# neevparikh/rpt

Hardware: AMD Instinct MI355X
Metric: Msamples/sec (higher is better)
Workload: dtype f32; 1 GPU; C3 lampshade-in-fog path trace 1024x1024x256spp; scene=examples/volumetric_pathtrace_lampshade.rs, parallelism=tile-shard x1, streams=2

## Files before the change

__graft_entry__.py:

```python
import os
import subprocess
import sys

ROOT = os.path.dirname(os.path.abspath(__file__))
if ROOT not in sys.path:
    sys.path.insert(0, ROOT)

HIPCC = os.environ.get("HIPCC", "/opt/rocm/bin/hipcc")
CSRC = os.path.join(ROOT, "rpt_amd", "csrc")
LIB = os.path.join(ROOT, "rpt_amd", "librpt_hip.so")


def _stale(target, sources):
    if not os.path.exists(target):
        return True
    t = os.path.getmtime(target)
    return any(os.path.getmtime(s) > t for s in sources)


def _digest(paths):
    import hashlib
    h = hashlib.sha256()
    for p in paths:
        with open(p, "rb") as f:
            h.update(f.read())
    return h.hexdigest()


SRCS = [os.path.join(CSRC, f) for f in ("kernels.hip", "kernels_f64.hip", "photon.hip", "rpt_capi.cpp", "rpt_comm.cpp")]
DEPS = SRCS + [os.path.join(CSRC, f) for f in ("device_core.h", "gpu_layout.h", "kernels.h", "host_internal.h", "f64_layout.h", "sort_scan.h")] + [
    os.path.join(ROOT, "include", "rpt_hip.h")]


FLAGS = ["--offload-arch=gfx950", "-O3", "-std=c++17", "-fno-slp-vectorize", "-fPIC", "-shared", "-Wl,-rpath,/opt/rocm/lib"]


FILE_FLAGS = {"kernels_f64.hip": ["-mllvm", "-disable-machine-licm"]}


def library_source_digest():
    import hashlib
    return hashlib.sha256((_digest(DEPS) + " ".join(FLAGS) + repr(sorted(FILE_FLAGS.items()))).encode()).hexdigest()


def _object_digest(src):
# ... 58 lines not shown
```

include/rpt_hip.h:

```cpp
#ifndef RPT_HIP_H
#define RPT_HIP_H

#include <stdint.h>

#ifdef __cplusplus
extern "C" {
#endif

#define RPT_OK 0
#define RPT_ERR_INVALID (-1)
#define RPT_ERR_STATE (-2)
#define RPT_ERR_DEVICE (-3)
#define RPT_ERR_UNSUPPORTED (-4)

typedef struct rpt_scene rpt_scene;

enum { RPT_SHAPE_SPHERE = 0, RPT_SHAPE_CUBE = 1, RPT_SHAPE_PLANE = 2, RPT_SHAPE_MESH = 3,
       RPT_SHAPE_GROUP = 4,
       RPT_SHAPE_MONOMIAL = 5  };

typedef struct rpt_shape_desc {
    int32_t kind;
    int32_t has_transform;
    double transform[16];
// ... 121 lines not shown
int rpt_debug_rng_u32(uint64_t seed, uint32_t pixel, uint32_t sample, uint32_t n, uint32_t* out);
int rpt_debug_material_sample_f(const rpt_material*, uint64_t n, const float* normals, const float* wos,
                                uint64_t seed, float* wi, float* pdf, int32_t* some);
int rpt_debug_material_bsdf(const rpt_material*, uint64_t n, const float* normals, const float* wos,
                            const float* wis, float* out_rgb);
int rpt_debug_radix_sort(uint64_t n, const uint64_t* keys, uint64_t* keys_out, uint32_t* order_out);
int rpt_debug_exclusive_scan2(uint64_t n, const uint32_t* a, const uint32_t* b, uint32_t* out_a, uint32_t* out_b, uint64_t totals[2]);
int rpt_debug_photon_positions64(rpt_scene*, double* out, uint64_t capacity);
int rpt_debug_photon_selections(rpt_scene*, uint32_t* out, uint64_t capacity_words, uint64_t dims[3]);
int rpt_debug_camera_rays(const rpt_camera*, const rpt_render_params*, uint64_t seed, uint32_t sample,
                          float* origins, float* dirs);
int rpt_debug_camera_sample(const rpt_camera*, const rpt_render_params*, uint64_t seed, uint32_t sample,
                            float* origins, float* dirs, uint32_t* next_word);
int rpt_debug_camera_sample_f64(const rpt_camera*, const rpt_render_params*, uint64_t seed, uint32_t sample,
                                double* origins, double* dirs, uint32_t* next_word);
int rpt_debug_light_sample(rpt_scene*, uint32_t light, uint64_t n, const float* positions, uint64_t seed, float* v, float* nrm,
                           float* pdf, float* intensity, float* wi, float* dist, uint32_t* next_word);
int rpt_debug_light_sample_f64(rpt_scene*, uint32_t light, uint64_t n, const double* positions, uint64_t seed, double* v, double* nrm,
                               double* pdf, double* intensity, double* wi, double* dist, uint32_t* next_word);
int rpt_debug_env_color(rpt_scene*, uint64_t n, const float* dirs, float* rgb);
int rpt_debug_env_color_f64(rpt_scene*, uint64_t n, const double* dirs, double* rgb);
int rpt_debug_medium_distance(rpt_scene*, uint64_t n, uint64_t seed, float* dmed, float* t_limit);
int rpt_debug_shadow_test(rpt_scene*, uint32_t light, uint64_t n, const float* origins, const float* dirs, const float* dist,
                          int32_t* out_flag, float* out_t);
int rpt_shadow_scan_info(rpt_scene*, uint32_t light, uint32_t out[4]);
int rpt_debug_distance_pair(float sigma_t, uint32_t k0, uint32_t n, float* out_new, float* out_guarded);

int rpt_debug_bounce(const rpt_material* m, uint32_t max_bounces, uint32_t depth, int32_t in_medium, int32_t medium_event,
                     float albedo_med, const float* medium_color, uint64_t n, const float* normals, const float* rds, uint64_t seed,
                     int32_t* flag, float* wi, float* k, uint32_t* next_word);
// ... 9 lines not shown
```

rpt_amd/_lib.py:

```python
import ctypes as C
import os
import sys

_HERE = os.path.dirname(os.path.abspath(__file__))
LIB_PATH = os.environ.get("RPT_LIB", os.path.join(_HERE, "librpt_hip.so"))


class RptError(RuntimeError):
    """Raised for every non-zero return code of the C ABI (message from rpt_last_error)."""


class ShapeDesc(C.Structure):
    pass


ShapeDesc._fields_ = [
    ("kind", C.c_int32),
    ("has_transform", C.c_int32),
    ("transform", C.c_double * 16),
    ("plane_normal", C.c_double * 3),
    ("plane_value", C.c_double),
    ("tris", C.POINTER(C.c_double)),
    ("n_tris", C.c_uint64),
    ("children", C.POINTER(ShapeDesc)),
# ... 105 lines not shown
     [C.POINTER(MaterialDesc), C.c_uint64, _P, _P, C.c_uint64, _P, _P, _P]),
    ("rpt_debug_material_bsdf", C.c_int, [C.POINTER(MaterialDesc), C.c_uint64, _P, _P, _P, _P]),
    ("rpt_debug_radix_sort", C.c_int, [C.c_uint64, _P, _P, _P]),
    ("rpt_debug_exclusive_scan2", C.c_int, [C.c_uint64, _P, _P, _P, _P, C.POINTER(C.c_uint64)]),
    ("rpt_debug_photon_positions64", C.c_int, [_P, _P, C.c_uint64]),
    ("rpt_debug_photon_selections", C.c_int, [_P, _P, C.c_uint64, C.POINTER(C.c_uint64)]),
    ("rpt_debug_camera_rays", C.c_int,
     [C.POINTER(CameraDesc), C.POINTER(RenderParams), C.c_uint64, C.c_uint32, _P, _P]),
    ("rpt_debug_light_sample", C.c_int, [_P, C.c_uint32, C.c_uint64, _P, C.c_uint64, _P, _P, _P, _P, _P, _P, _P]),
    ("rpt_debug_light_sample_f64", C.c_int, [_P, C.c_uint32, C.c_uint64, _P, C.c_uint64, _P, _P, _P, _P, _P, _P, _P]),
    ("rpt_debug_env_color", C.c_int, [_P, C.c_uint64, _P, _P]),
    ("rpt_debug_env_color_f64", C.c_int, [_P, C.c_uint64, _P, _P]),
    ("rpt_debug_medium_distance", C.c_int, [_P, C.c_uint64, C.c_uint64, _P, _P]),
    ("rpt_debug_camera_sample", C.c_int,
     [C.POINTER(CameraDesc), C.POINTER(RenderParams), C.c_uint64, C.c_uint32, _P, _P, _P]),
    ("rpt_debug_camera_sample_f64", C.c_int,
     [C.POINTER(CameraDesc), C.POINTER(RenderParams), C.c_uint64, C.c_uint32, _P, _P, _P]),
    ("rpt_debug_bounce", C.c_int, [C.POINTER(MaterialDesc), C.c_uint32, C.c_uint32, C.c_int32, C.c_int32, C.c_float, _P,
                                   C.c_uint64, _P, _P, C.c_uint64, _P, _P, _P, _P]),
    ("rpt_debug_shadow_test", C.c_int, [_P, C.c_uint32, C.c_uint64, _P, _P, _P, _P, _P]),
    ("rpt_debug_distance_pair", C.c_int, [C.c_float, C.c_uint32, C.c_uint32, _P, _P]),
    ("rpt_shadow_scan_info", C.c_int, [_P, C.c_uint32, C.POINTER(C.c_uint32)]),
    ("rpt_debug_material_f64", C.c_int, [C.POINTER(MaterialDesc), C.c_uint64, _P, _P, C.c_uint64, _P, _P, _P, _P, _P]),
    ("rpt_debug_material_bsdf_f64", C.c_int, [C.POINTER(MaterialDesc), C.c_uint64, _P, _P, _P, _P]),
]

_lib = None


def vp(a):
# ... 28 lines not shown
```

rpt_amd/api.py:

```python
import ctypes as C
import math
import weakref

import numpy as np

from . import _lib
from ._lib import RptError, vp as _vp

def shard_pixels(width, height, rank, count):
    lib = _lib.load()
    n = _lib.check(lib.rpt_shard_tiles(width, height, rank, count, None, 0))
    tiles = np.zeros(max(n, 1), dtype=np.uint32)
    _lib.check(lib.rpt_shard_tiles(width, height, rank, count, tiles.ctypes.data_as(C.c_void_p), n))
    tiles_x = (width + 31) // 32
    ys, xs = np.mgrid[0:32, 0:32]
    out = []
    for t in tiles[:n]:
        x = (int(t) % tiles_x) * 32 + xs
        y = (int(t) // tiles_x) * 32 + ys
        m = (x < width) & (y < height)
        out.append((y[m] * width + x[m]).astype(np.uint32))
    return np.sort(np.concatenate(out)) if out else np.zeros(0, dtype=np.uint32)


# ... 900 lines not shown
        o = np.ascontiguousarray(origins, dtype=np.float32).reshape(-1, 3)
        d = np.ascontiguousarray(dirs, dtype=np.float32).reshape(-1, 3)
        ds = np.ascontiguousarray(dist, dtype=np.float32).reshape(-1)
        n = o.shape[0]
        if d.shape[0] != n or ds.shape[0] != n:
            raise ValueError("origins, dirs and dist differ in length")
        flag, t = np.empty(n, np.int32), np.empty(n, np.float32)
        _lib.check(lib.rpt_debug_shadow_test(h, light_index, n, _vp(o), _vp(d), _vp(ds), _vp(flag), _vp(t)))
        return flag, t

    def shadow_scan_info(self, light_index):
        out = (C.c_uint32 * 4)()
        _lib.check(_lib.load().rpt_shadow_scan_info(self.scene._commit(self.device_), light_index, out))
        return {"twin_lo": int(out[0]), "twin_hi": int(out[1]), "shadow_form": int(out[2]), "twin_object": int(np.int32(np.uint32(out[3])))}


def debug_distance_pair(sigma_t, k0, n):
    new, guarded = np.empty(n, np.float32), np.empty(n, np.float32)
    _lib.check(_lib.load().rpt_debug_distance_pair(float(sigma_t), int(k0), int(n), _vp(new), _vp(guarded)))
    return new, guarded


def debug_bounce(material, normals, rds, max_bounces=3, depth=0, seed=0, in_medium=False, medium_event=False, albedo_med=0.0,
                 medium_color=(0.0, 0.0, 0.0)):
    nrm = np.ascontiguousarray(normals, dtype=np.float32).reshape(-1, 3)
    rd = np.ascontiguousarray(rds, dtype=np.float32).reshape(-1, 3)
    n = nrm.shape[0]
    if rd.shape[0] != n:
        raise ValueError("normals and rds differ in length")
    mcol = np.ascontiguousarray(medium_color, dtype=np.float32).reshape(3)
# ... 29 lines not shown
    md = material_desc(material, _lib.MaterialDesc)
    _lib.check(_lib.load().rpt_debug_material_bsdf_f64(C.byref(md), n, *[_vp(a) for a in arrs], _vp(f)))
    return f


def debug_camera_sample(camera, width, height, sample=0, seed=0, f64=False):
    ft = np.float64 if f64 else np.float32
    n = width * height
    out = {"o": np.empty((n, 3), ft), "d": np.empty((n, 3), ft), "next_word": np.empty(n, np.uint32)}
    prm = _lib.RenderParams(width, height, 0.0, 0, 0, 1)
    lib = _lib.load()
    fn = lib.rpt_debug_camera_sample_f64 if f64 else lib.rpt_debug_camera_sample
    _lib.check(fn(C.byref(camera_desc(camera, _lib.CameraDesc)), C.byref(prm), seed, sample,
                  *[_vp(out[k]) for k in ("o", "d", "next_word")]))
    return out
```

rpt_amd/csrc/kernels.h:

```cpp
#pragma once
#include <hip/hip_runtime_api.h>
#include <stddef.h>
#include <stdint.h>
#include "gpu_layout.h"

namespace rptg {

struct RenderArgs {
    SceneView sc;
    CameraG cam;
    uint32_t width, height;
    float inv_dim;
    uint32_t max_bounces;
    uint32_t iterations;
    uint32_t sample_offset;
    uint32_t chunk_spp;
    uint32_t n_chunks;
    uint64_t seed_mixed;
    const uint32_t* tiles;
    uint32_t n_tiles, tiles_x;
    uint32_t n_owned;
    uint32_t n_items;
    float* slab;
    float* slab2;
    unsigned long long* queue;
    unsigned long long* counters;
    uint32_t lds_stack;
    uint32_t defer_lanes;
    uint32_t defer_stop;
    uint32_t walk_leaf_quarters;
    uint32_t detach;
    uint32_t pull_batch;
    uint32_t detach_trigger;
    uint32_t stream_backlog;
    uint32_t stream_contexts;
    uint32_t n_twin_lights;
    uint32_t* stream_scratch;
};

static_assert(offsetof(RenderArgs, sc) == 0, "RenderArgs must begin with the SceneView");

struct KernelInfo {
// ... 15 lines not shown
hipError_t launch_frame_unpack(const double* d_packed, double* d_frame, const uint32_t* d_tiles, uint32_t n_tiles, uint32_t tiles_x,
                               uint32_t width, uint32_t height, hipStream_t st);
__attribute__((weak)) hipError_t launch_intersect_segments(const SceneView& sc, uint64_t n, const float* d_o, const float* d_d, const float* d_tmax,
                                                           float* d_t, uint32_t* d_code, hipStream_t stream);
hipError_t launch_intersect(const SceneView& sc, uint64_t n, const float* d_o, const float* d_d, float* d_t,
                            int32_t* d_obj, float* d_n, bool bvh, hipStream_t stream);
hipError_t launch_debug_rng(uint64_t seed_mixed, uint32_t pixel, uint32_t sample, uint32_t n, uint32_t* d_out,
                            hipStream_t stream);
hipError_t launch_debug_sample_f(const Material& m, uint64_t n, const float* d_n, const float* d_wo,
                                 uint64_t seed_mixed, float* d_wi, float* d_pdf, int32_t* d_some, hipStream_t s);
hipError_t launch_debug_bsdf(const Material& m, uint64_t n, const float* d_n, const float* d_wo, const float* d_wi,
                             float* d_out, hipStream_t s);
__attribute__((weak)) hipError_t launch_debug_camera_sample(const CameraG& cam, uint32_t w, uint32_t h, float inv_dim, uint64_t seed_mixed,
                                                            uint32_t sample, float* d_o, float* d_d, uint32_t* d_next_word ,
                                                            hipStream_t s);
struct LightSampleArgs {
    uint32_t light;
    uint32_t pad_;
    uint64_t n;
    uint64_t seed_mixed;
    const float* pos;
    float *v, *nrm, *pdf;
    float *intensity, *wi, *dist;
    uint32_t* next_word;
};
__attribute__((weak)) hipError_t launch_debug_light_sample(const SceneView& sc, const LightSampleArgs& q, hipStream_t s);
__attribute__((weak)) hipError_t launch_debug_env_color(const SceneView& sc, uint64_t n, const float* d_dirs, float* d_rgb, hipStream_t s);
__attribute__((weak)) hipError_t launch_debug_medium_distance(const SceneView& sc, uint64_t n, uint64_t seed_mixed, float* d_dmed,
                                                              float* d_limit, hipStream_t s);
struct ShadowTestArgs {
// ... 38 lines not shown
```

rpt_amd/csrc/kernels.hip:

```cpp
#include "device_core.h"
#include "kernels.h"

namespace rptg {

RPT_DEV uint32_t mbcnt64(uint64_t m) {
    return __builtin_amdgcn_mbcnt_hi(uint32_t(m >> 32), __builtin_amdgcn_mbcnt_lo(uint32_t(m), 0u));
}
template <bool MONO = false>
RPT_DEV uint32_t code_object(const SceneView& sc, uint32_t code, uint32_t inst) {
    uint32_t kind = code >> 28, idx = code & 0x0FFFFFFFu;
    float w;
    if (MONO && kind == K_MONO) w = sc.mono_sh[idx].r0.w;
    else if (kind == K_INSTTRI) w = sc.inst[inst].n0.w;
    else if (kind == K_SPHERE) w = sc.sph_sh[idx].r0.w;
    else if (kind == K_CUBE) w = sc.cub_sh[idx].r0.w;
    else if (kind == K_PLANE) w = sc.pln_sh[idx].unit_n_obj.w;
    else if (kind == K_TRI) w = sc.tri_sh[idx].n1.w;
    else if (kind == K_AABB) w = sc.aabb[idx].lo.w;
    else if (kind == K_RECT) w = sc.rect_sh[idx].n_obj.w;
    else w = sc.btri_sh[idx].n1.w;
    return __float_as_uint(w);
}
RPT_DEV float ray_tmin(V o) { return 2e-5f * (1.f + max3(fabsf(o.x), fabsf(o.y), fabsf(o.z))); }

// ... 181 lines not shown
        if (bounce) {
            float pdf;
            SECT(13);
            const V wo = -normalize(rd);
            bounce = sample_f(mat, n, wo, rng, wi, pdf);
            if (bounce) {
                V f = bsdf(mat, n, wo, wi);
                float wgt = fabsf(dot(wi, n)) * rcp(MEDIUM ? pdf * 0.8f : pdf);
                k = wgt * f;
            }
        }
    }
    return bounce && !is_zero(k);
}

template <bool MEDIUM, int BVH, bool COUNT, bool GROUPS = false, int DETACH = 0, bool MONO = false>
__global__ __launch_bounds__(256, BVH == 0 ? ((GROUPS || COUNT || MONO) ? RPT_MIN_WAVES_SCAN_GROUPS : RPT_MIN_WAVES_SCAN) : BVH == 3 ? RPT_MIN_WAVES_SCENE_MESH : BVH == 1 ? (DETACH == 2 ? RPT_MIN_WAVES_STREAM : RPT_MIN_WAVES_MESH) : RPT_MIN_WAVES)
void render_kernel(const RenderArgs a) {
#ifdef RPT_SECT_CLOCKS
    __shared__ unsigned long long sect_lds_[4][56];
    if ((threadIdx.x & 63u) < 56u) sect_lds_[threadIdx.x >> 6][threadIdx.x & 63u] = 0ull;
    uint64_t sect_clk_ = __builtin_amdgcn_s_memtime();
    uint32_t sect_prev_ = 27u;
#endif
    static_assert(DETACH == 0 || (MEDIUM && BVH == 1 && !GROUPS), "detached tree walks: per-mesh-tree kernels in a medium only");
    static_assert(DETACH == 0 || !MONO, "no detached tree walks in scenes with monomial surfaces");
    extern __shared__ uint32_t dyn_lds[];
    const SceneView& sc = a.sc;
    uint32_t* stk = BVH ? (dyn_lds + threadIdx.x) : nullptr;
    const uint32_t stride = 256;

    const float sigma_t = sc.sigma_a + sc.sigma_s;
    const float inv_sigma_t = MEDIUM ? 1.f / sigma_t : 0.f;
    const float albedo_med = MEDIUM ? sc.sigma_s / sigma_t : 0.f;

    Rng rng;
    rng.s0 = rng.s1 = rng.s2 = rng.s3 = 0;
    V ro = mk(0, 0, 0), rd = mk(0, 0, 1);
    V P = mk(0, 0, 0), Q = mk(1, 1, 1), Rc = mk(kInf, kInf, kInf);
    constexpr uint32_t kStackRows = BVH == 1 ? (DETACH ? kDetachStackRows : 21u) : 32u;
    constexpr uint32_t kStateBase = BVH ? kStackRows * 256u : 0u;
    uint32_t* const ls = dyn_lds + kStateBase + threadIdx.x;
    enum { S_SLAB = 0, S_END = 1, S_PIX = 2, S_XN = 3, S_YN = 4, S_S = 5, S_ACC = 6, S_P = 9, S_Q = 12, S_RC = 15, S_ROWS = 18 };
    static_assert(S_RC + 3 == S_ROWS, "the staged tables begin right behind the state rows");
    constexpr uint32_t kTabBase = kStateBase + (BVH == 0 ? uint32_t(S_ROWS) : 5u) * 256u;
    LdsTables tab;
    {
        const F4* const t4 = reinterpret_cast<const F4*>(dyn_lds + kTabBase);
        F4* const w4 = reinterpret_cast<F4*>(dyn_lds + kTabBase);
        const uint32_t nm = sc.n_obj <= kLdsMats ? sc.n_obj : 0u, nl = sc.n_ltris <= kLdsLtris ? sc.n_ltris : 0u;
        for (uint32_t i = threadIdx.x; i < 2u * nm; i += 256u) w4[i] = reinterpret_cast<const F4*>(sc.mats)[i];
        for (uint32_t i = threadIdx.x; i < 6u * nl; i += 256u) w4[2u * kLdsMats + i] = reinterpret_cast<const F4*>(sc.ltris)[i];
        __syncthreads();
        tab.mats = t4; tab.n_mats = nm;
        tab.ltris = t4 + 2u * kLdsMats; tab.n_ltris = nl;
    }
    auto in_lds = [](int k) { return BVH == 0 || k <= S_YN; };
    V acc_r = mk(0, 0, 0);
    uint32_t slab_idx_r = 0, s_r = 0, s_end_r = 0, pix_r = 0;
// ... 87 lines not shown
        const uint32_t n_want = uint32_t(__popcll(__ballot(want)));
        if (n_want != 0u && (n_want >= a.pull_batch || __ballot(alive && !want) == 0ull)) {
            const auto& ka = *kernarg_args<RenderArgs>();
            SECTK(0);
            if (want && have_item) {
                if constexpr (DETACH) {
                    const volatile unsigned long long* av = acc64;
                    reinterpret_cast<float4*>(ka.slab)[ldu(S_SLAB, slab_idx_r)] =
                        make_float4(from_fixed(av[threadIdx.x]), from_fixed(av[256u + threadIdx.x]), from_fixed(av[512u + threadIdx.x]), 0.f);
                } else {
                    reinterpret_cast<float4*>(ka.slab)[ldu(S_SLAB, slab_idx_r)] =
                        make_float4(ldf(S_ACC + 0, acc_r.x), ldf(S_ACC + 1, acc_r.y), ldf(S_ACC + 2, acc_r.z), 0.f);
                }
                have_item = false;
            }
            for (;;) {
                const uint64_t m = __ballot(want);
                if (m == 0) break;
                if (pool_next == pool_end) {
                    unsigned long long base = ~0ull;
                    if (first_batch) {
                        base = (unsigned long long)(blockIdx.x * 4u + (threadIdx.x >> 6)) * 64ull;
                        first_batch = false;
                    } else if (!drained && (threadIdx.x & 63u) == 0) {
                        base = atomicAdd(ka.queue, 64ull);
                    }
                    const uint32_t lo = __builtin_amdgcn_readfirstlane(uint32_t(base));
                    const uint32_t hi = __builtin_amdgcn_readfirstlane(uint32_t(base >> 32));
                    if (hi != 0 || lo >= ka.n_items) {
                        drained = true;
                        if (want) alive = false;
                        break;
                    }
                    pool_next = lo;
                    pool_end = min(lo + 64u, ka.n_items);
                    pool_chunk = lo / ka.n_owned;
                    const uint32_t p0 = lo - pool_chunk * ka.n_owned;
// ... 14 lines not shown
                    if (x < ka.width && y < ka.height) {
                        want = false;
                        have_item = true;
                        item_done = false;
                        stu(S_SLAB, slab_idx_r, item);
                        if constexpr (DETACH) {
                            volatile unsigned long long* av = acc64;
                            av[threadIdx.x] = 0ull; av[256u + threadIdx.x] = 0ull; av[512u + threadIdx.x] = 0ull;
                        } else {
                            stf(S_ACC + 0, acc_r.x, 0.f);
                            stf(S_ACC + 1, acc_r.y, 0.f);
                            stf(S_ACC + 2, acc_r.z, 0.f);
                        }
                        const uint32_t s0 = chunk * ka.chunk_spp;
                        stu(S_S, s_r, s0);
                        stu(S_END, s_end_r, min(s0 + ka.chunk_spp, ka.iterations));
                        stu(S_PIX, pix_r, y * ka.width + x);
                        stf(S_XN, xn_r, pixel_xn(x, ka.width, ka.inv_dim));
                        stf(S_YN, yn_r, pixel_yn(y, ka.height, ka.inv_dim));
                    }
                }
            }
        }
        if (need_path && alive && !item_done && !(DETACH == 2 && uint32_t(__popc(parked_mask)) >= a.stream_contexts)) {
            if (alive) {
                const auto& ka = *kernarg_args<RenderArgs>();
                SECTK(1);
                const uint32_t s = ldu(S_S, s_r);
                rng.seed(ka.seed_mixed, ldu(S_PIX, pix_r), ka.sample_offset + s);
                float dx = rng.range(-ka.inv_dim, ka.inv_dim);
                float dy = rng.range(-ka.inv_dim, ka.inv_dim);
                const CameraG cam = kernarg_load(&ka.cam);
                cast_ray(cam, ldf(S_XN, xn_r) + dx, ldf(S_YN, yn_r) + dy, rng, ro, rd);
                depth = 0;
                if constexpr (BVH == 0) {
                    stv(S_P, P, mk(0, 0, 0));
                    stv(S_Q, Q, mk(1, 1, 1));
                    if (!MEDIUM) stv(S_RC, Rc, mk(kInf, kInf, kInf));
                } else {
                    P = mk(0, 0, 0);
                    Q = mk(1, 1, 1);
                    Rc = mk(kInf, kInf, kInf);
                }
                stu(S_S, s_r, s + 1u);
                item_done = s + 1u >= ldu(S_END, s_end_r);
                need_path = false;
                if (DETACH == 2) { phase = PH_NEW; did_work = true; }
                if (COUNT) c_samples++;
// ... 904 lines not shown
__global__ void debug_bsdf_kernel(const Material m, uint64_t n, const float* nrm, const float* wo, const float* wi,
                                  float* out) {
    uint64_t i = uint64_t(blockIdx.x) * blockDim.x + threadIdx.x;
    if (i >= n) return;
    V f = bsdf(mat_from(m), mk(nrm[3 * i], nrm[3 * i + 1], nrm[3 * i + 2]), mk(wo[3 * i], wo[3 * i + 1], wo[3 * i + 2]),
               mk(wi[3 * i], wi[3 * i + 1], wi[3 * i + 2]));
    out[3 * i] = f.x; out[3 * i + 1] = f.y; out[3 * i + 2] = f.z;
}
__global__ void debug_camera_kernel(const CameraG cam, uint32_t w, uint32_t h, float inv_dim, uint64_t seed_mixed, uint32_t sample,
                                    float* o, float* d, uint32_t* next_word) {
    uint32_t i = blockIdx.x * blockDim.x + threadIdx.x;
    if (i >= w * h) return;
    uint32_t x = i % w, y = i / w;
    float xn = pixel_xn(x, w, inv_dim);
    float yn = pixel_yn(y, h, inv_dim);
    Rng r;
    r.seed(seed_mixed, i, sample);
    float dx = r.range(-inv_dim, inv_dim);
    float dy = r.range(-inv_dim, inv_dim);
    V ro, rd;
    cast_ray(cam, xn + dx, yn + dy, r, ro, rd);
    o[3 * i] = ro.x; o[3 * i + 1] = ro.y; o[3 * i + 2] = ro.z;
    d[3 * i] = rd.x; d[3 * i + 1] = rd.y; d[3 * i + 2] = rd.z;
    if (next_word) next_word[i] = r.next();
}
template <bool GROUPS>
__global__ __launch_bounds__(256) void debug_light_sample_kernel(const SceneView sc, const LightSampleArgs q) {
    __shared__ F4 lds_ltris[6u * kLdsLtris];
    LdsTables tab;
    {
        const uint32_t nl = sc.n_ltris <= kLdsLtris ? sc.n_ltris : 0u;
        for (uint32_t i = threadIdx.x; i < 6u * nl; i += 256u) lds_ltris[i] = reinterpret_cast<const F4*>(sc.ltris)[i];
        __syncthreads();
        tab.ltris = lds_ltris; tab.n_ltris = nl;
    }
    const uint64_t i = uint64_t(blockIdx.x) * 256u + threadIdx.x;
    if (i >= q.n) return;
    const Light L = uload(&sc.lights[q.light]);
    const V pos = mk(q.pos[3 * i], q.pos[3 * i + 1], q.pos[3 * i + 2]);
// ... 58 lines not shown
    if (i >= q.n) return;
    Rng r;
    r.seed(q.seed_mixed, uint32_t(i), 0);
    V wi = mk(0.f, 0.f, 0.f), k = mk(0.f, 0.f, 0.f);
    const bool go = stage_bounce<MEDIUM, false>(a, q.albedo_med, mk(q.rd[3 * i], q.rd[3 * i + 1], q.rd[3 * i + 2]), q.depth,
                                                MEDIUM && q.medium_event != 0u, mk(q.nrm[3 * i], q.nrm[3 * i + 1], q.nrm[3 * i + 2]),
                                                mk(q.mcol[0], q.mcol[1], q.mcol[2]), mat_from(q.m), r, wi, k);
    q.flag[i] = go ? 1 : 0;
    q.wi[3 * i] = wi.x; q.wi[3 * i + 1] = wi.y; q.wi[3 * i + 2] = wi.z;
    q.k[3 * i] = k.x; q.k[3 * i + 1] = k.y; q.k[3 * i + 2] = k.z;
    q.next_word[i] = r.next();
}

static constexpr size_t kStackBytes = 32u * 256u * sizeof(uint32_t);
static constexpr size_t kTabBytes = (2u * 32u + 6u * 8u) * 16u;
static constexpr size_t kStateBytes = 18u * 256u * sizeof(uint32_t) + kTabBytes;
static constexpr size_t kStateBytesBvh = 5u * 256u * sizeof(uint32_t) + kTabBytes;
static constexpr size_t kMeshTreeBytes = (21u + 5u) * 256u * sizeof(uint32_t) + kTabBytes;
static constexpr size_t kDetachBytes = kDetachDwords * sizeof(uint32_t);
static_assert(kTabBytes == kTabDwords * 4u, "one table layout");

template <bool M, int B, bool C>
static hipError_t launch_render_t(const RenderArgs& a, int n_blocks, hipStream_t stream) {
    const size_t lds = B == 1 ? kMeshTreeBytes : B ? kStackBytes + kStateBytesBvh : kStateBytes;
    if (a.sc.n_mono) {
        if (a.sc.n_lparts) hipLaunchKernelGGL((render_kernel<M, B, false, true, 0, true>), dim3(n_blocks), dim3(256), lds, stream, a);
        else hipLaunchKernelGGL((render_kernel<M, B, false, false, 0, true>), dim3(n_blocks), dim3(256), lds, stream, a);
        return hipGetLastError();
    }
    if constexpr (M && B == 1) {
#ifdef RPT_EXPERIMENTS
// ... 99 lines not shown
    hipLaunchKernelGGL(debug_sample_f_kernel, dim3(uint32_t((n + 255) / 256)), dim3(256), 0, s, m, n, d_n, d_wo, seed_mixed,
                       d_wi, d_pdf, d_some);
    return hipGetLastError();
}
hipError_t launch_debug_bsdf(const Material& m, uint64_t n, const float* d_n, const float* d_wo, const float* d_wi,
                             float* d_out, hipStream_t s) {
    hipLaunchKernelGGL(debug_bsdf_kernel, dim3(uint32_t((n + 255) / 256)), dim3(256), 0, s, m, n, d_n, d_wo, d_wi, d_out);
    return hipGetLastError();
}
hipError_t launch_debug_camera_sample(const CameraG& cam, uint32_t w, uint32_t h, float inv_dim, uint64_t seed_mixed, uint32_t sample,
                                      float* d_o, float* d_d, uint32_t* d_next_word, hipStream_t s) {
    hipLaunchKernelGGL(debug_camera_kernel, dim3((w * h + 255) / 256), dim3(256), 0, s, cam, w, h, inv_dim, seed_mixed, sample, d_o, d_d,
                       d_next_word);
    return hipGetLastError();
}
hipError_t launch_debug_light_sample(const SceneView& sc, const LightSampleArgs& q, hipStream_t s) {
    const dim3 grid(uint32_t((q.n + 255) / 256));
    if (sc.n_lparts) hipLaunchKernelGGL(debug_light_sample_kernel<true>, grid, dim3(256), 0, s, sc, q);
    else hipLaunchKernelGGL(debug_light_sample_kernel<false>, grid, dim3(256), 0, s, sc, q);
    return hipGetLastError();
}
hipError_t launch_debug_env_color(const SceneView& sc, uint64_t n, const float* d_dirs, float* d_rgb, hipStream_t s) {
    hipLaunchKernelGGL(debug_env_color_kernel, dim3(uint32_t((n + 255) / 256)), dim3(256), 0, s, sc, n, d_dirs, d_rgb);
    return hipGetLastError();
}
hipError_t launch_debug_medium_distance(const SceneView& sc, uint64_t n, uint64_t seed_mixed, float* d_dmed, float* d_limit,
                                        hipStream_t s) {
    hipLaunchKernelGGL(debug_medium_distance_kernel, dim3(uint32_t((n + 255) / 256)), dim3(256), 0, s, sc, n, seed_mixed, d_dmed, d_limit);
    return hipGetLastError();
}
// ... 21 lines not shown
```

rpt_amd/csrc/rpt_capi.cpp:

```cpp
#include <hip/hip_runtime_api.h>

#include <algorithm>
#include <cfloat>
#include <cmath>
#include <cstdio>
#include <cstring>
#include <functional>
#include <limits>
#include <memory>
#include <mutex>
#include <string>
#include <unordered_map>
#include <vector>

#include "../../include/rpt_hip.h"
#include "host_internal.h"
#include "kernels.h"
#include "f64_layout.h"

using namespace rptg;

static thread_local std::string g_err;
namespace rpti {
int fail(int code, const std::string& msg) {
// ... 18 lines not shown
        hipError_t e__ = (expr);                                                                   \
        if (e__ != hipSuccess)                                                                     \
            return fail(RPT_ERR_DEVICE, std::string(#expr) + ": " + hipGetErrorString(e__));       \
    } while (0)

struct rpt_options {
    int64_t counters = 0;
    int64_t chunk_spp = 0;
    int64_t blocks_per_cu = 0;
    int64_t max_blocks = 0;
    int64_t timing = 0;
    int64_t room_shell = 1;
    int64_t scan_specialise = 1;
    int64_t scan_cull = 1;
    int64_t shadow_scan = 1;
    int64_t photon_skip = 0;
    int64_t photon_block_lists = 1;
    int64_t photon_coop_gather = 1;
    int64_t photon_split = 0;
    int64_t photon_parts = 4;
    int64_t instancing = 1;
    int64_t bvh_leaf_max = 4;
    int64_t bvh_max_depth = 20;
    int64_t bvh_sweep_below = 4096;
    int64_t defer_stop = 16;
    int64_t walk_leaf_quarters = 6;
    int64_t defer_lanes = 32;
    int64_t detach_shadows = 1;
    int64_t stream_backlog = 48;
    int64_t stream_contexts = 1;
// ... 10 lines not shown
};
static rpt_options g_defaults;
static std::mutex g_defaults_mutex;
static int set_option_in(rpt_options& o, const char* name, int64_t value) {
    if (!name) return fail(RPT_ERR_INVALID, "null option name");
    const std::string s(name);
    if (s == "counters") o.counters = value;
    else if (s == "chunk_spp") { if (value < 0) return fail(RPT_ERR_INVALID, "chunk_spp must be >= 0 (0 = auto)"); o.chunk_spp = value; }
    else if (s == "blocks_per_cu") o.blocks_per_cu = value;
    else if (s == "max_blocks") { if (value < 0 || value > (1 << 20)) return fail(RPT_ERR_INVALID, "max_blocks must be 0..2^20 (0 = no cap)"); o.max_blocks = value; }
    else if (s == "timing") o.timing = value;
    else if (s == "room_shell") o.room_shell = value;
    else if (s == "scan_specialise") o.scan_specialise = value;
    else if (s == "scan_cull") o.scan_cull = value;
    else if (s == "shadow_scan") o.shadow_scan = value;
    else if (s == "photon_skip") o.photon_skip = value;
    else if (s == "photon_block_lists") o.photon_block_lists = value;
    else if (s == "photon_parts") o.photon_parts = value;
    else if (s == "photon_split") {
#ifndef RPT_EXPERIMENTS
        if (value != 0) return fail(RPT_ERR_UNSUPPORTED, "photon_split: a rejected prototype, built with -DRPT_EXPERIMENTS only");
#endif
        o.photon_split = value;
    }
    else if (s == "photon_coop_gather") o.photon_coop_gather = value;
    else if (s == "instancing") o.instancing = value;
    else if (s == "defer_lanes") { if (value < 1 || value > 64) return fail(RPT_ERR_INVALID, "defer_lanes must be 1..64"); o.defer_lanes = value; }
    else if (s == "bvh_leaf_max") { if (value < 1 || value > 16) return fail(RPT_ERR_INVALID, "bvh_leaf_max must be 1..16"); o.bvh_leaf_max = value; }
    else if (s == "bvh_sweep_below") { if (value < 0) return fail(RPT_ERR_INVALID, "bvh_sweep_below must be >= 0"); o.bvh_sweep_below = value; }
    else if (s == "bvh_max_depth") { if (value < 1 || value > 20) return fail(RPT_ERR_INVALID, "bvh_max_depth must be 1..20"); o.bvh_max_depth = value; }
// ... 380 lines not shown
    struct Device {
        rpti::DevMem arena;
        rpti::DevMem arena64;
        rpti::DevMem d_tiles;
        LaunchSet sets[2];
        rpti::DevMem d_counters;
        rpti::DevMem d_out;
        std::vector<rpti::Event> evs;
    } dev;
    int cur_set = 0;
    uint64_t last_counters[64] = {0};
    uint64_t last_cull[12] = {0};
    static constexpr size_t kTimedLaunches = 1024;
    size_t ev_count = 0;
    int last_blocks = 0;
    uint64_t prims_per_ray = 0;
    uint32_t n_twin_lights = 0;
    std::vector<Light> light_records;
    bool twins_scanned = false;
    uint64_t stats[16] = {0};
    void* photon = nullptr;
    rpt64::Scene view64{};
    double medium_color64[3] = {0, 0, 0}, medium_color_hi64[3] = {0, 0, 0};
    const rpt64::MeshNode* mnodes64 = nullptr;
    const uint32_t* mleaf64 = nullptr;
    const uint32_t* mroot64 = nullptr;
    uint64_t mesh_tree_info64[8] = {0};
    uint64_t last_counters64[64] = {0};
    std::unordered_map<uint64_t, std::vector<std::shared_ptr<const std::vector<double>>>> mesh_pool;
    uint32_t tk_w = 0, tk_h = 0, tk_rank = 0, tk_count = 0, n_tiles = 0, tiles_x = 0;
// ... 1833 lines not shown
    a.tiles_x = s->tiles_x;
    a.n_owned = a.n_tiles * 1024u;
    uint64_t n_items = uint64_t(a.n_owned) * a.n_chunks;
    if (n_items >= (1ull << 32) - (1ull << 24)) return fail(RPT_ERR_INVALID, "too many work items; raise chunk_spp");
    a.n_items = uint32_t(n_items);
    size_t slab_bytes = std::max<size_t>(size_t(n_items) * slab_item_bytes, 16);
    if (s->dev.sets[s->cur_set].used && s->dev.sets[s->cur_set].stream != st) s->cur_set ^= 1;
    rpt_scene::LaunchSet& ls = s->dev.sets[s->cur_set];
    if (ls.used && ls.stream != st) HIP_TRY(hipStreamWaitEvent(st, ls.done.get(), 0));
    HIP_TRY(ls.d_slab.reserve(slab_bytes));
    ls.stream = st;
    ls.used = true;
    a.slab = ls.d_slab.get<float>();
    a.queue = ls.d_queue.get<unsigned long long>();
    a.counters = s->opt.counters ? s->dev.d_counters.get<unsigned long long>() : nullptr;
    a.lds_stack = s->view.n_nodes ? 1u : 0u;
    a.defer_lanes = uint32_t(s->opt.defer_lanes);
    a.defer_stop = uint32_t(std::min(s->opt.defer_stop, s->opt.defer_lanes));
    a.walk_leaf_quarters = uint32_t(s->opt.walk_leaf_quarters);
    a.detach = 0;
    if (s->opt.detach_shadows && s->view.has_medium && bvh_mode(s->view) == 1 && s->view.n_lparts == 0 && s->twins_scanned)
        a.detach = (s->opt.detach_shadows == 2 && s->n_twin_lights <= 3) ? 2u : 1u;
    a.stream_backlog = uint32_t(s->opt.stream_backlog);
    a.stream_contexts = uint32_t(s->opt.stream_contexts);
    a.n_twin_lights = s->n_twin_lights;
    a.stream_scratch = nullptr;
    a.pull_batch = uint32_t(s->opt.pull_batch);
    a.detach_trigger = uint32_t(s->opt.detach_trigger);
    if (a.detach) {
        a.defer_lanes = uint32_t(s->opt.detach_lanes);
        a.defer_stop = uint32_t(std::min<int64_t>(s->opt.defer_stop, std::min(s->opt.detach_lanes, s->opt.detach_trigger)));
// ... 49 lines not shown
    HIP_TRY(hipEventRecord(mine.done.get(), st));
    return RPT_OK;
}
static int run_render(rpt_scene* s, const rpt_render_params* prm, const RenderArgs& a_in, double* d_out, hipStream_t st) {
    RenderArgs a = a_in;
    int bpc = int(s->opt.blocks_per_cu);
    if (bpc <= 0) {
        HIP_TRY(render_occupancy(a.sc.has_medium != 0, bvh_mode(a.sc), &bpc, int(a.detach)));
        if (bpc < 1) bpc = 1;
    }
    if (a.detach == 2) {
        rpt_scene::LaunchSet& ls = s->dev.sets[s->dev.sets[0].d_queue.get() == a.queue ? 0 : 1];
        HIP_TRY(ls.d_stream.reserve(size_t(s->n_cus) * size_t(bpc) * stream_scratch_bytes_per_block()));
        a.stream_scratch = ls.d_stream.get<uint32_t>();
    }
    return rpti::run_persistent(s, prm, a, d_out, st, bpc,
                                [](const RenderArgs& ra, int nb, hipStream_t stream) { return launch_render(ra, nb, stream); }, true);
}
extern "C++" rpti::SceneDev rpti::scene_dev(rpt_scene* s) {
    int first = -1;
    for (size_t i = 0; i < s->lights.size(); i++)
        if (s->lights[i].kind == L_OBJECT) { first = int(i); break; }
    bool mono = false;
    for (const auto& o : s->objects) mono = mono || holds_monomial(o.shape);
    return SceneDev{s->committed, s->device, s->n_cus, s->view, first, bool(s->dev.arena64), mono};
}
extern "C++" void*& rpti::photon_slot(rpt_scene* s) { return s->photon; }
extern "C++" int64_t rpti::option_photon_skip(rpt_scene* s) { return s->opt.photon_skip; }
extern "C++" int64_t rpti::option_max_blocks(rpt_scene* s) { return s->opt.max_blocks; }
extern "C++" int64_t rpti::option_f64_photon_slice(rpt_scene* s) { return s->opt.f64_photon_slice; }
// ... 325 lines not shown
}
int rpt_debug_material_bsdf(const rpt_material* m, uint64_t n, const float* normals, const float* wos, const float* wis,
                            float* out_rgb) {
    std::string why;
    if (!check_material(m, why) || !normals || !wos || !wis || !out_rgb) return fail(RPT_ERR_INVALID, "bad argument");
    rpti::DevMem d_n, d_wo, d_wi, d_out;
    HIP_TRY(hook_scratch(d_n, n * 12));
    HIP_TRY(hook_scratch(d_wo, n * 12));
    HIP_TRY(hook_scratch(d_wi, n * 12));
    HIP_TRY(hook_scratch(d_out, n * 12));
    HIP_TRY(hipMemcpy(d_n.get(), normals, n * 12, hipMemcpyHostToDevice));
    HIP_TRY(hipMemcpy(d_wo.get(), wos, n * 12, hipMemcpyHostToDevice));
    HIP_TRY(hipMemcpy(d_wi.get(), wis, n * 12, hipMemcpyHostToDevice));
    HIP_TRY(launch_debug_bsdf(to_gpu_material(m), n, d_n.get<float>(), d_wo.get<float>(), d_wi.get<float>(), d_out.get<float>(), nullptr));
    HIP_TRY(hipMemcpy(out_rgb, d_out.get(), n * 12, hipMemcpyDeviceToHost));
    return RPT_OK;
}
int rpt_debug_camera_sample(const rpt_camera* cam, const rpt_render_params* prm, uint64_t seed, uint32_t sample,
                            float* origins, float* dirs, uint32_t* next_word) {
    if (!cam || !prm || !origins || !dirs) return fail(RPT_ERR_INVALID, "null argument");
    if (prm->width == 0 || prm->height == 0) return fail(RPT_ERR_INVALID, "empty frame");
    if (uint64_t(prm->width) * prm->height > (1ull << 31)) return fail(RPT_ERR_INVALID, "image too large");
    if (!launch_debug_camera_sample) return fail(RPT_ERR_UNSUPPORTED, "rpt_debug_camera_sample: built without the kernels");
    const size_t n = size_t(prm->width) * prm->height;
    rpti::DevMem d_o, d_d, d_w;
    HIP_TRY(hook_scratch(d_o, n * 12));
    HIP_TRY(hook_scratch(d_d, n * 12));
    if (next_word) HIP_TRY(hook_scratch(d_w, n * 4));
    HIP_TRY(launch_debug_camera_sample(camera_g(cam), prm->width, prm->height, inv_dim_of(prm), seed_mix(seed), sample, d_o.get<float>(),
                                       d_d.get<float>(), next_word ? d_w.get<uint32_t>() : nullptr, nullptr));
// ... 172 lines not shown
```

Baseline: 14850 Msamples/s.

## Pregenerate camera rays and RNG states per chunk across the wave

When a wave takes new pixel chunks in the scan (BVH==0) path, it cooperatively generates camera-sample RNG states and ray directions for every sample in each received chunk. Lanes spread the tasks evenly and write the results to per-wave global scratch, and each later sample start loads its state instead of seeding and casting inline. The aim is to stop divergent lanes from idling during camera ray generation, since lanes otherwise refill at different times. In exchange it adds scratch traffic, two extra LDS rows and a fence, and it is enabled by default for non-thin-lens cameras with chunk_spp up to 32.

Measured after the change: 13980 Msamples/s. 5.9% lower.

```diff
diff --git a/__graft_entry__.py b/__graft_entry__.py
--- a/__graft_entry__.py
+++ b/__graft_entry__.py
@@ -28,7 +28,7 @@
 
 
 SRCS = [os.path.join(CSRC, f) for f in ("kernels.hip", "kernels_f64.hip", "photon.hip", "rpt_capi.cpp", "rpt_comm.cpp")]
-DEPS = SRCS + [os.path.join(CSRC, f) for f in ("device_core.h", "gpu_layout.h", "kernels.h", "host_internal.h", "f64_layout.h", "sort_scan.h")] + [
+DEPS = SRCS + [os.path.join(CSRC, f) for f in ("device_core.h", "gpu_layout.h", "kernels.h", "host_internal.h", "f64_layout.h", "sort_scan.h", "sample_pregen.h")] + [
     os.path.join(ROOT, "include", "rpt_hip.h")]
 
 
diff --git a/include/rpt_hip.h b/include/rpt_hip.h
--- a/include/rpt_hip.h
+++ b/include/rpt_hip.h
@@ -159,6 +159,9 @@
                             float* origins, float* dirs, uint32_t* next_word);
 int rpt_debug_camera_sample_f64(const rpt_camera*, const rpt_render_params*, uint64_t seed, uint32_t sample,
                                 double* origins, double* dirs, uint32_t* next_word);
+int rpt_sample_pregen_info(rpt_scene*, uint64_t out[4]);
+int rpt_debug_sample_states(const rpt_camera*, const rpt_render_params*, uint64_t seed, uint32_t iterations, uint32_t sample_offset,
+                            uint32_t sample, float* dirs, uint32_t* words);
 int rpt_debug_light_sample(rpt_scene*, uint32_t light, uint64_t n, const float* positions, uint64_t seed, float* v, float* nrm,
                            float* pdf, float* intensity, float* wi, float* dist, uint32_t* next_word);
 int rpt_debug_light_sample_f64(rpt_scene*, uint32_t light, uint64_t n, const double* positions, uint64_t seed, double* v, double* nrm,
diff --git a/rpt_amd/_lib.py b/rpt_amd/_lib.py
--- a/rpt_amd/_lib.py
+++ b/rpt_amd/_lib.py
@@ -143,6 +143,9 @@
     ("rpt_debug_medium_distance", C.c_int, [_P, C.c_uint64, C.c_uint64, _P, _P]),
     ("rpt_debug_camera_sample", C.c_int,
      [C.POINTER(CameraDesc), C.POINTER(RenderParams), C.c_uint64, C.c_uint32, _P, _P, _P]),
+    ("rpt_sample_pregen_info", C.c_int, [_P, C.POINTER(C.c_uint64)]),
+    ("rpt_debug_sample_states", C.c_int,
+     [C.POINTER(CameraDesc), C.POINTER(RenderParams), C.c_uint64, C.c_uint32, C.c_uint32, C.c_uint32, _P, _P]),
     ("rpt_debug_camera_sample_f64", C.c_int,
      [C.POINTER(CameraDesc), C.POINTER(RenderParams), C.c_uint64, C.c_uint32, _P, _P, _P]),
     ("rpt_debug_bounce", C.c_int, [C.POINTER(MaterialDesc), C.c_uint32, C.c_uint32, C.c_int32, C.c_int32, C.c_float, _P,
diff --git a/rpt_amd/api.py b/rpt_amd/api.py
--- a/rpt_amd/api.py
+++ b/rpt_amd/api.py
@@ -938,6 +938,11 @@
         _lib.check(_lib.load().rpt_shadow_scan_info(self.scene._commit(self.device_), light_index, out))
         return {"twin_lo": int(out[0]), "twin_hi": int(out[1]), "shadow_form": int(out[2]), "twin_object": int(np.int32(np.uint32(out[3])))}
 
+    def sample_pregen_info(self):
+        out = (C.c_uint64 * 4)()
+        _lib.check(_lib.load().rpt_sample_pregen_info(self.scene._commit(self.device_), out))
+        return {"stored": int(out[0]), "chunk_spp": int(out[1]), "scratch_bytes": int(out[2]), "option": int(out[3])}
+
 
 def debug_distance_pair(sigma_t, k0, n):
     new, guarded = np.empty(n, np.float32), np.empty(n, np.float32)
@@ -997,3 +1002,13 @@
     _lib.check(fn(C.byref(camera_desc(camera, _lib.CameraDesc)), C.byref(prm), seed, sample,
                   *[_vp(out[k]) for k in ("o", "d", "next_word")]))
     return out
+
+
+
+def debug_sample_states(camera, width, height, iterations, sample, sample_offset=0, seed=0):
+    n = width * height
+    out = {"d": np.empty((n, 3), np.float32), "words": np.empty((n, 4), np.uint32)}
+    prm = _lib.RenderParams(width, height, 0.0, 0, 0, 1)
+    _lib.check(_lib.load().rpt_debug_sample_states(C.byref(camera_desc(camera, _lib.CameraDesc)), C.byref(prm), seed, iterations,
+                                                    sample_offset, sample, _vp(out["d"]), _vp(out["words"])))
+    return out
diff --git a/rpt_amd/csrc/kernels.h b/rpt_amd/csrc/kernels.h
--- a/rpt_amd/csrc/kernels.h
+++ b/rpt_amd/csrc/kernels.h
@@ -3,6 +3,7 @@
 #include <stddef.h>
 #include <stdint.h>
 #include "gpu_layout.h"
+#include "sample_pregen.h"
 
 namespace rptg {
 
@@ -25,7 +26,7 @@
     float* slab2;
     unsigned long long* queue;
     unsigned long long* counters;
-    uint32_t lds_stack;
+    uint32_t sample_magic;
     uint32_t defer_lanes;
     uint32_t defer_stop;
     uint32_t walk_leaf_quarters;
@@ -71,6 +72,7 @@
 __attribute__((weak)) hipError_t launch_debug_camera_sample(const CameraG& cam, uint32_t w, uint32_t h, float inv_dim, uint64_t seed_mixed,
                                                             uint32_t sample, float* d_o, float* d_d, uint32_t* d_next_word ,
                                                             hipStream_t s);
+__attribute__((weak)) hipError_t launch_debug_sample_states(const RenderArgs& a, uint32_t sample, float* d_dirs, uint32_t* d_words, hipStream_t s);
 struct LightSampleArgs {
     uint32_t light;
     uint32_t pad_;
diff --git a/rpt_amd/csrc/kernels.hip b/rpt_amd/csrc/kernels.hip
--- a/rpt_amd/csrc/kernels.hip
+++ b/rpt_amd/csrc/kernels.hip
@@ -219,6 +219,60 @@
     return bounce && !is_zero(k);
 }
 
+enum { S_SLAB = 0, S_END = 1, S_PIX = 2, S_XN = 3, S_YN = 4, S_S = 5, S_ACC = 6, S_P = 9, S_Q = 12, S_RC = 15, S_TBL = 18, S_S0 = 19, S_ROWS = 20 };
+RPT_DEV uint32_t sample_tid() {
+    uint32_t tid = threadIdx.x;
+    asm volatile("" : "+v"(tid));
+    return tid;
+}
+RPT_DEV char* sample_wave_base(uint32_t cs, uint32_t tid) {
+    const auto& ka = *kernarg_args<RenderArgs>();
+    const uint32_t wave = blockIdx.x * 4u + __builtin_amdgcn_readfirstlane(tid >> 6);
+    return reinterpret_cast<char*>(ka.stream_scratch) + size_t(wave) * (64u * kSampleStateDwords * 4u) * cs;
+}
+RPT_DEV void sample_pass(uint32_t* rows, bool recv, uint64_t rm) {
+    const auto& ka = *kernarg_args<RenderArgs>();
+    const uint32_t tid = sample_tid();
+    uint32_t* const col0 = rows + (tid & ~63u);
+    if (recv) col0[S_TBL * 256 + mbcnt64(rm)] = tid & 63u;
+    __builtin_amdgcn_fence(__ATOMIC_RELEASE, "workgroup");
+    const uint32_t cs = ka.chunk_spp, magic = ka.sample_magic, n_tasks = uint32_t(__popcll(rm)) * cs;
+    char* const wbase = sample_wave_base(cs, tid);
+    const CameraG cam = kernarg_load(&ka.cam);
+    for (uint32_t t0 = 0u; t0 < n_tasks; t0 += 64u) {
+        const uint32_t t = t0 + (tid & 63u);
+        if (t < n_tasks) {
+            uint32_t r, j;
+            sample_task_split(t, cs, magic, r, j);
+            const uint32_t owner = col0[S_TBL * 256 + r];
+            const uint32_t* const oc = col0 + owner;
+            const uint32_t s = oc[S_S0 * 256] + j;
+            if (s < oc[S_END * 256]) {
+                Rng g;
+                g.seed(ka.seed_mixed, oc[S_PIX * 256], ka.sample_offset + s);
+                const float dx = g.range(-ka.inv_dim, ka.inv_dim);
+                const float dy = g.range(-ka.inv_dim, ka.inv_dim);
+                V o, d;
+                cast_ray(cam, __uint_as_float(oc[S_XN * 256]) + dx, __uint_as_float(oc[S_YN * 256]) + dy, g, o, d);
+                u4v* const slot = reinterpret_cast<u4v*>(wbase + (owner * cs + j) * (kSampleStateDwords * 4u));
+                slot[0] = u4v{g.s0, g.s1, g.s2, g.s3};
+                slot[1] = u4v{__float_as_uint(d.x), __float_as_uint(d.y), __float_as_uint(d.z), 0u};
+            }
+        }
+    }
+    __builtin_amdgcn_fence(__ATOMIC_RELEASE, "workgroup");
+}
+RPT_DEV void sample_load(uint32_t j, Rng& rng, V& ro, V& rd) {
+    const auto& ka = *kernarg_args<RenderArgs>();
+    const uint32_t cs = ka.chunk_spp;
+    const uint32_t tid = sample_tid();
+    const u4v* const slot = reinterpret_cast<const u4v*>(sample_wave_base(cs, tid) + ((tid & 63u) * cs + j) * (kSampleStateDwords * 4u));
+    const u4v w0 = __builtin_nontemporal_load(slot), w1 = __builtin_nontemporal_load(slot + 1);
+    rng.s0 = w0.x; rng.s1 = w0.y; rng.s2 = w0.z; rng.s3 = w0.w;
+    rd = mk(__uint_as_float(w1.x), __uint_as_float(w1.y), __uint_as_float(w1.z));
+    ro = mk(ka.cam.eye[0], ka.cam.eye[1], ka.cam.eye[2]);
+}
+
 template <bool MEDIUM, int BVH, bool COUNT, bool GROUPS = false, int DETACH = 0, bool MONO = false>
 __global__ __launch_bounds__(256, BVH == 0 ? ((GROUPS || COUNT || MONO) ? RPT_MIN_WAVES_SCAN_GROUPS : RPT_MIN_WAVES_SCAN) : BVH == 3 ? RPT_MIN_WAVES_SCENE_MESH : BVH == 1 ? (DETACH == 2 ? RPT_MIN_WAVES_STREAM : RPT_MIN_WAVES_MESH) : RPT_MIN_WAVES)
 void render_kernel(const RenderArgs a) {
@@ -246,8 +300,7 @@
     constexpr uint32_t kStackRows = BVH == 1 ? (DETACH ? kDetachStackRows : 21u) : 32u;
     constexpr uint32_t kStateBase = BVH ? kStackRows * 256u : 0u;
     uint32_t* const ls = dyn_lds + kStateBase + threadIdx.x;
-    enum { S_SLAB = 0, S_END = 1, S_PIX = 2, S_XN = 3, S_YN = 4, S_S = 5, S_ACC = 6, S_P = 9, S_Q = 12, S_RC = 15, S_ROWS = 18 };
-    static_assert(S_RC + 3 == S_ROWS, "the staged tables begin right behind the state rows");
+    static_assert(S_S0 + 1 == S_ROWS, "the staged tables begin right behind the state rows");
     constexpr uint32_t kTabBase = kStateBase + (BVH == 0 ? uint32_t(S_ROWS) : 5u) * 256u;
     LdsTables tab;
     {
@@ -365,13 +418,14 @@
                 }
                 have_item = false;
             }
+            bool recv = false;
             for (;;) {
                 const uint64_t m = __ballot(want);
                 if (m == 0) break;
                 if (pool_next == pool_end) {
                     unsigned long long base = ~0ull;
                     if (first_batch) {
-                        base = (unsigned long long)(blockIdx.x * 4u + (threadIdx.x >> 6)) * 64ull;
+                        base = (unsigned long long)(blockIdx.x * 4u + ((BVH == 0 ? sample_tid() : threadIdx.x) >> 6)) * 64ull;
                         first_batch = false;
                     } else if (!drained && (threadIdx.x & 63u) == 0) {
                         base = atomicAdd(ka.queue, 64ull);
@@ -416,11 +470,20 @@
                         }
                         const uint32_t s0 = chunk * ka.chunk_spp;
                         stu(S_S, s_r, s0);
+                        if constexpr (BVH == 0) ls[S_S0 * 256] = s0;
+                        recv = true;
                         stu(S_END, s_end_r, min(s0 + ka.chunk_spp, ka.iterations));
                         stu(S_PIX, pix_r, y * ka.width + x);
                         stf(S_XN, xn_r, pixel_xn(x, ka.width, ka.inv_dim));
                         stf(S_YN, yn_r, pixel_yn(y, ka.height, ka.inv_dim));
                     }
+                }
+            }
+            if constexpr (BVH == 0) {
+                const uint64_t rm = __ballot(recv);
+                if (ka.sample_magic != 0u && rm != 0ull) {
+                    SECTK(23);
+                    sample_pass(dyn_lds + kStateBase, recv, rm);
                 }
             }
         }
@@ -429,11 +492,17 @@
                 const auto& ka = *kernarg_args<RenderArgs>();
                 SECTK(1);
                 const uint32_t s = ldu(S_S, s_r);
-                rng.seed(ka.seed_mixed, ldu(S_PIX, pix_r), ka.sample_offset + s);
-                float dx = rng.range(-ka.inv_dim, ka.inv_dim);
-                float dy = rng.range(-ka.inv_dim, ka.inv_dim);
-                const CameraG cam = kernarg_load(&ka.cam);
-                cast_ray(cam, ldf(S_XN, xn_r) + dx, ldf(S_YN, yn_r) + dy, rng, ro, rd);
+                bool stored = false;
+                if constexpr (BVH == 0) stored = ka.sample_magic != 0u;
+                if (stored) {
+                    if constexpr (BVH == 0) sample_load(s - ls[S_S0 * 256], rng, ro, rd);
+                } else {
+                    rng.seed(ka.seed_mixed, ldu(S_PIX, pix_r), ka.sample_offset + s);
+                    float dx = rng.range(-ka.inv_dim, ka.inv_dim);
+                    float dy = rng.range(-ka.inv_dim, ka.inv_dim);
+                    const CameraG cam = kernarg_load(&ka.cam);
+                    cast_ray(cam, ldf(S_XN, xn_r) + dx, ldf(S_YN, yn_r) + dy, rng, ro, rd);
+                }
                 depth = 0;
                 if constexpr (BVH == 0) {
                     stv(S_P, P, mk(0, 0, 0));
@@ -1368,6 +1437,7 @@
     uint32_t x = i % w, y = i / w;
     float xn = pixel_xn(x, w, inv_dim);
     float yn = pixel_yn(y, h, inv_dim);
+    asm volatile("" : "+v"(xn), "+v"(yn));
     Rng r;
     r.seed(seed_mixed, i, sample);
     float dx = r.range(-inv_dim, inv_dim);
@@ -1377,6 +1447,30 @@
     o[3 * i] = ro.x; o[3 * i + 1] = ro.y; o[3 * i + 2] = ro.z;
     d[3 * i] = rd.x; d[3 * i + 1] = rd.y; d[3 * i + 2] = rd.z;
     if (next_word) next_word[i] = r.next();
+}
+__global__ __launch_bounds__(256) void debug_sample_states_kernel(const RenderArgs a, uint32_t sample, float* __restrict__ d, uint32_t* __restrict__ words) {
+    __shared__ uint32_t rows[S_ROWS * 256];
+    const uint32_t i = blockIdx.x * 256u + threadIdx.x;
+    const bool recv = i < a.width * a.height;
+    const uint32_t s0 = sample / a.chunk_spp * a.chunk_spp;
+    if (recv) {
+        uint32_t* const ls = rows + threadIdx.x;
+        const uint32_t x = i % a.width, y = i / a.width;
+        ls[S_S0 * 256] = s0;
+        ls[S_END * 256] = min(s0 + a.chunk_spp, a.iterations);
+        ls[S_PIX * 256] = i;
+        ls[S_XN * 256] = __float_as_uint(pixel_xn(x, a.width, a.inv_dim));
+        ls[S_YN * 256] = __float_as_uint(pixel_yn(y, a.height, a.inv_dim));
+    }
+    const uint64_t rm = __ballot(recv);
+    if (rm == 0ull) return;
+    sample_pass(rows, recv, rm);
+    if (!recv) return;
+    Rng r;
+    V ro, rd;
+    sample_load(sample - s0, r, ro, rd);
+    d[3 * i] = rd.x; d[3 * i + 1] = rd.y; d[3 * i + 2] = rd.z;
+    for (uint32_t k = 0; k < 4u; k++) words[4 * i + k] = r.next();
 }
 template <bool GROUPS>
 __global__ __launch_bounds__(256) void debug_light_sample_kernel(const SceneView sc, const LightSampleArgs q) {
@@ -1465,7 +1559,7 @@
 
 static constexpr size_t kStackBytes = 32u * 256u * sizeof(uint32_t);
 static constexpr size_t kTabBytes = (2u * 32u + 6u * 8u) * 16u;
-static constexpr size_t kStateBytes = 18u * 256u * sizeof(uint32_t) + kTabBytes;
+static constexpr size_t kStateBytes = 20u * 256u * sizeof(uint32_t) + kTabBytes;
 static constexpr size_t kStateBytesBvh = 5u * 256u * sizeof(uint32_t) + kTabBytes;
 static constexpr size_t kMeshTreeBytes = (21u + 5u) * 256u * sizeof(uint32_t) + kTabBytes;
 static constexpr size_t kDetachBytes = kDetachDwords * sizeof(uint32_t);
@@ -1595,6 +1689,10 @@
                        d_next_word);
     return hipGetLastError();
 }
+hipError_t launch_debug_sample_states(const RenderArgs& a, uint32_t sample, float* d_dirs, uint32_t* d_words, hipStream_t s) {
+    hipLaunchKernelGGL(debug_sample_states_kernel, dim3((a.width * a.height + 255u) / 256u), dim3(256), 0, s, a, sample, d_dirs, d_words);
+    return hipGetLastError();
+}
 hipError_t launch_debug_light_sample(const SceneView& sc, const LightSampleArgs& q, hipStream_t s) {
     const dim3 grid(uint32_t((q.n + 255) / 256));
     if (sc.n_lparts) hipLaunchKernelGGL(debug_light_sample_kernel<true>, grid, dim3(256), 0, s, sc, q);
diff --git a/rpt_amd/csrc/rpt_capi.cpp b/rpt_amd/csrc/rpt_capi.cpp
--- a/rpt_amd/csrc/rpt_capi.cpp
+++ b/rpt_amd/csrc/rpt_capi.cpp
@@ -56,6 +56,7 @@
     int64_t scan_specialise = 1;
     int64_t scan_cull = 1;
     int64_t shadow_scan = 1;
+    int64_t sample_pregen = 1;
     int64_t photon_skip = 0;
     int64_t photon_block_lists = 1;
     int64_t photon_coop_gather = 1;
@@ -96,6 +97,7 @@
     else if (s == "scan_specialise") o.scan_specialise = value;
     else if (s == "scan_cull") o.scan_cull = value;
     else if (s == "shadow_scan") o.shadow_scan = value;
+    else if (s == "sample_pregen") { if (value < 0 || value > 1) return fail(RPT_ERR_INVALID, "sample_pregen must be 0 or 1"); o.sample_pregen = value; }
     else if (s == "photon_skip") o.photon_skip = value;
     else if (s == "photon_block_lists") o.photon_block_lists = value;
     else if (s == "photon_parts") o.photon_parts = value;
@@ -506,6 +508,7 @@
     static constexpr size_t kTimedLaunches = 1024;
     size_t ev_count = 0;
     int last_blocks = 0;
+    uint64_t last_pregen[4] = {0};
     uint64_t prims_per_ray = 0;
     uint32_t n_twin_lights = 0;
     std::vector<Light> light_records;
@@ -2369,7 +2372,7 @@
     a.slab = ls.d_slab.get<float>();
     a.queue = ls.d_queue.get<unsigned long long>();
     a.counters = s->opt.counters ? s->dev.d_counters.get<unsigned long long>() : nullptr;
-    a.lds_stack = s->view.n_nodes ? 1u : 0u;
+    a.sample_magic = 0u;
     a.defer_lanes = uint32_t(s->opt.defer_lanes);
     a.defer_stop = uint32_t(std::min(s->opt.defer_stop, s->opt.defer_lanes));
     a.walk_leaf_quarters = uint32_t(s->opt.walk_leaf_quarters);
@@ -2449,6 +2452,17 @@
         HIP_TRY(ls.d_stream.reserve(size_t(s->n_cus) * size_t(bpc) * stream_scratch_bytes_per_block()));
         a.stream_scratch = ls.d_stream.get<uint32_t>();
     }
+    s->last_pregen[0] = s->last_pregen[2] = 0;
+    s->last_pregen[1] = a.chunk_spp;
+    if (s->opt.sample_pregen && bvh_mode(a.sc) == 0 && !(a.cam.aperture > 0.f) && a.chunk_spp <= kSampleChunkMax) {
+        rpt_scene::LaunchSet& ls = s->dev.sets[s->dev.sets[0].d_queue.get() == a.queue ? 0 : 1];
+        const size_t bytes = sample_scratch_bytes(uint32_t(s->n_cus), uint32_t(bpc), a.chunk_spp);
+        HIP_TRY(ls.d_stream.reserve(bytes));
+        a.stream_scratch = ls.d_stream.get<uint32_t>();
+        a.sample_magic = sample_task_magic(a.chunk_spp);
+        s->last_pregen[0] = 1;
+        s->last_pregen[2] = bytes;
+    }
     return rpti::run_persistent(s, prm, a, d_out, st, bpc,
                                 [](const RenderArgs& ra, int nb, hipStream_t stream) { return launch_render(ra, nb, stream); }, true);
 }
@@ -2804,6 +2818,46 @@
     HIP_TRY(hipMemcpy(d_wi.get(), wis, n * 12, hipMemcpyHostToDevice));
     HIP_TRY(launch_debug_bsdf(to_gpu_material(m), n, d_n.get<float>(), d_wo.get<float>(), d_wi.get<float>(), d_out.get<float>(), nullptr));
     HIP_TRY(hipMemcpy(out_rgb, d_out.get(), n * 12, hipMemcpyDeviceToHost));
+    return RPT_OK;
+}
+int rpt_sample_pregen_info(rpt_scene* s, uint64_t out[4]) {
+    if (!s || !out) return fail(RPT_ERR_INVALID, "null argument");
+    for (int i = 0; i < 3; i++) out[i] = s->last_pregen[i];
+    out[3] = uint64_t(s->opt.sample_pregen);
+    return RPT_OK;
+}
+int rpt_debug_sample_states(const rpt_camera* cam, const rpt_render_params* prm, uint64_t seed, uint32_t iterations, uint32_t sample_offset,
+                            uint32_t sample, float* dirs, uint32_t* words) {
+    if (!cam || !prm || !dirs || !words) return fail(RPT_ERR_INVALID, "null argument");
+    if (prm->width == 0 || prm->height == 0 || uint64_t(prm->width) * prm->height > (1ull << 20)) return fail(RPT_ERR_INVALID, "rpt_debug_sample_states: 1..2^20 pixels");
+    if (sample >= iterations) return fail(RPT_ERR_INVALID, "rpt_debug_sample_states: sample >= iterations");
+    if (cam->aperture > 0.0) return fail(RPT_ERR_UNSUPPORTED, "rpt_debug_sample_states: a thin-lens camera has no stored samples");
+    if (!launch_debug_sample_states) return fail(RPT_ERR_UNSUPPORTED, "rpt_debug_sample_states: built without the kernels");
+    int64_t opt;
+    {
+        std::lock_guard<std::mutex> lock(g_defaults_mutex);
+        opt = g_defaults.chunk_spp;
+    }
+    RenderArgs a{};
+    a.cam = camera_g(cam);
+    a.width = prm->width;
+    a.height = prm->height;
+    a.inv_dim = inv_dim_of(prm);
+    a.iterations = iterations;
+    a.sample_offset = sample_offset;
+    a.chunk_spp = chunk_rule(opt, iterations, 0, 0);
+    if (a.chunk_spp > kSampleChunkMax) return fail(RPT_ERR_INVALID, "rpt_debug_sample_states: chunk_spp above 32");
+    a.seed_mixed = seed_mix(seed);
+    a.sample_magic = sample_task_magic(a.chunk_spp);
+    const size_t n = size_t(prm->width) * prm->height;
+    rpti::DevMem d_s, d_d, d_w;
+    HIP_TRY(hook_scratch(d_s, sample_scratch_bytes(uint32_t((n + 255) / 256), 1, a.chunk_spp)));
+    HIP_TRY(hook_scratch(d_d, n * 12));
+    HIP_TRY(hook_scratch(d_w, n * 16));
+    a.stream_scratch = d_s.get<uint32_t>();
+    HIP_TRY(launch_debug_sample_states(a, sample, d_d.get<float>(), d_w.get<uint32_t>(), nullptr));
+    HIP_TRY(hipMemcpy(dirs, d_d.get(), n * 12, hipMemcpyDeviceToHost));
+    HIP_TRY(hipMemcpy(words, d_w.get(), n * 16, hipMemcpyDeviceToHost));
     return RPT_OK;
 }
 int rpt_debug_camera_sample(const rpt_camera* cam, const rpt_render_params* prm, uint64_t seed, uint32_t sample,
diff --git a/rpt_amd/csrc/sample_pregen.h b/rpt_amd/csrc/sample_pregen.h
--- /dev/null
+++ b/rpt_amd/csrc/sample_pregen.h
@@ -0,0 +1,26 @@
+#pragma once
+#include <stddef.h>
+#include <stdint.h>
+
+#if defined(__HIP__)
+#define RPT_SP_HD __host__ __device__ inline
+#else
+#define RPT_SP_HD inline
+#endif
+
+namespace rptg {
+
+static constexpr uint32_t kSampleChunkMax = 32u;
+static constexpr uint32_t kSampleTaskMax = 64u * kSampleChunkMax;
+static constexpr uint32_t kSampleStateDwords = 8u;
+
+RPT_SP_HD uint32_t sample_task_magic(uint32_t chunk_spp) { return (65536u + chunk_spp - 1u) / chunk_spp; }
+RPT_SP_HD void sample_task_split(uint32_t t, uint32_t chunk_spp, uint32_t magic, uint32_t& r, uint32_t& j) {
+    r = (t * magic) >> 16;
+    j = t - r * chunk_spp;
+}
+RPT_SP_HD size_t sample_scratch_bytes(uint32_t n_cus, uint32_t blocks_per_cu, uint32_t chunk_spp) {
+    return size_t(n_cus) * blocks_per_cu * 4u * 64u * chunk_spp * (kSampleStateDwords * 4u);
+}
+
+}
```
